# Lichtso/contrast_renderer

Hardware: AMD Instinct MI355X
Metric: paths/sec, 10k mixed-Bezier paths @ 4096^2 (tessellate + tile raster) (higher is better)
Workload: dtype f32

## Files before the change

contrast_renderer_amd/build.py:

```python
import os
import subprocess
import sys

HERE = os.path.dirname(os.path.abspath(__file__))
CSRC = os.path.join(HERE, "csrc")
SOURCES = ("tessellate.hip", "raster.hip", "bin_edges.hip", "raster_edges.hip", "image_filter.hip", "api.hip", "image.hip", "comm.hip", "text.cpp", "path.cpp")
FLAGS = ["--offload-arch=gfx950", "-O3", "-std=c++17", "-ffp-contract=off", "-fno-fast-math", "-fPIC", "-Wall", "-Wno-unused-function", "-Wno-bitwise-instead-of-logical"]
FILE_FLAGS = {"raster_edges.hip": ["-fno-slp-vectorize"], "bin_edges.hip": ["-fno-slp-vectorize", "-mllvm", "-disable-machine-licm"], "raster.hip": ["-fno-slp-vectorize", "-mllvm", "-pragma-unroll-threshold=65536"], "tessellate.hip": ["-fno-slp-vectorize"]}
OUT = os.path.join(HERE, "libcontrast_hip.so")


def _newer(target, deps):
    if not os.path.exists(target):
        return False
    t = os.path.getmtime(target)
    return all(os.path.getmtime(d) <= t for d in deps if os.path.exists(d))


def header_deps():
    own = sorted(os.path.join(CSRC, f) for f in os.listdir(CSRC) if f.endswith((".hpp", ".h", ".inc")))
    return own + [os.path.join(HERE, "..", "include", h) for h in ("contrast_hip.h", "crh_fmath.h")]


def file_flags():
# ... 18 lines not shown
        objects.append(obj)
        if not force and _newer(obj, [os.path.join(CSRC, src)] + headers):
            continue
        flags = (FLAGS + os.environ.get("CRH_EXTRA_FLAGS", "").split()) if src.endswith(".hip") else [f for f in FLAGS if not f.startswith("--offload-arch")]
        flags = flags + file_flags().get(src, [])
        cmd = [hipcc] + flags + ["-c", os.path.join(CSRC, src), "-o", obj]
        if verbose:
            print(" ".join(cmd), file=sys.stderr)
        procs.append((src, subprocess.Popen(cmd, stdout=subprocess.PIPE, stderr=subprocess.STDOUT)))
    for src, proc in procs:
        out, _ = proc.communicate()
        if proc.returncode != 0:
            raise RuntimeError(f"hipcc failed on {src}:\n{out.decode()}")
        if verbose and out:
            print(out.decode(), file=sys.stderr)
    exports = write_export_map()
    if procs or not os.path.exists(OUT) or os.path.getmtime(exports) > os.path.getmtime(OUT):
        cmd = [hipcc, "--offload-arch=gfx950", "-shared", "-fPIC"] + objects + ["-ldl", "-Wl,--version-script=" + exports, "-o", OUT]
        subprocess.check_call(cmd)
    return OUT


DEBUG_TAPS = ("crh_debug_frame_counters", "crh_debug_frame_counters16", "crh_debug_frame_words", "crh_debug_frame_bin_dump", "crh_debug_flat_batches", "crh_debug_pass_leaves_state",
              "crh_debug_frame_last_pass")


def declared_entry_points():
    import re
    with open(os.path.join(HERE, "..", "include", "contrast_hip.h")) as f:
        return sorted(set(re.findall(r"\b(crh_[a-z_0-9]+)\s*\(", f.read())) - {"crh_status"})


def write_export_map():
    path = os.path.join(HERE, "build", "exports.map")
    os.makedirs(os.path.dirname(path), exist_ok=True)
    text = "{\n  global:\n" + "".join(f"    {name};\n" for name in declared_entry_points() + list(DEBUG_TAPS)) + "  local:\n    *;\n};\n"
    if not os.path.exists(path) or open(path).read() != text:
        with open(path, "w") as f:
            f.write(text)
    return path


if __name__ == "__main__":
    print(build_library(force="--force" in sys.argv, verbose=True))
```

contrast_renderer_amd/csrc/api.hip:

```cpp
#include <hip/hip_runtime.h>

#include <algorithm>
#include <atomic>
#include <chrono>
#include <cmath>
#include <cstdio>
#include <cstdlib>
#include <cstring>
#include <memory>
#include <string>
#include <vector>

#include "api_internal.hpp"
#include "launch.hpp"
#include "raster_params.hpp"
#include "scene.hpp"

using namespace crh;

namespace {
thread_local std::string g_error;

struct DevBuf {
    void* p = nullptr;
// ... 2604 lines not shown
    return CRH_OK;
}
extern "C" crh_status crh_debug_frame_last_pass(crh_frame* f, uint32_t out[4]) {
    if (!f || !out) return CRH_ERR_INVALID_ARGUMENT;
    out[0] = f->last_formulation, out[1] = f->last_general, out[2] = f->last_raster, out[3] = f->last_bin;
    const crh_frame::BinSet& set = f->sets[f->last_set];
    if ((f->last_bin & kBinReplayed) && set.used && set.flags_host && hipEventQuery(set.flags_ready) == hipSuccess && set.flags_host[kReplayFallbackWord] != 0u) out[3] |= kBinFellBack;
    return CRH_OK;
}
extern "C" crh_status crh_debug_frame_words(crh_frame* f, uint32_t out[128]) {
    HIP_TRY(hipSetDevice(f->renderer->device));
    HIP_TRY(f->renderer->sync());
    HIP_TRY(hipMemcpy(out, f->sets[f->last_set].overflow_p, 512, hipMemcpyDeviceToHost));
    HIP_TRY(hipMemset(static_cast<uint8_t*>(f->sets[f->last_set].overflow_p) + 320, 0, 192));
    return CRH_OK;
}
extern "C" crh_status crh_debug_frame_bin_dump(crh_frame* f, uint32_t* out, uint32_t n_words) {
    HIP_TRY(hipSetDevice(f->renderer->device));
    HIP_TRY(f->renderer->sync());
    if ((size_t)n_words * 4 > f->item_cost.cap) return CRH_ERR_INVALID_ARGUMENT;
    HIP_TRY(hipMemcpy(out, f->item_cost.p, (size_t)n_words * 4, hipMemcpyDeviceToHost));
    return CRH_OK;
}
extern "C" int crh_debug_flat_batches(const uint32_t* cost, uint32_t n_items, uint32_t* runs, uint32_t cap_runs, uint32_t limits[4]) {
    std::vector<uint32_t> out;
    flat_batches(cost, n_items, out);
    flat_batch_limits(n_items, limits);
    if (out.size() / 2 > cap_runs) return -1;
    std::copy(out.begin(), out.end(), runs);
    return (int)(out.size() / 2);
}
crh_status crh_frame_device_pointer(crh_frame* f, void** out) {
    if (!f || !out) return CRH_ERR_INVALID_ARGUMENT;
    crh_status st = settle_frame(f);
    if (st != CRH_OK) return st;
    HIP_TRY(hipSetDevice(f->renderer->device));
    HIP_TRY(order_after_external(f, f->renderer->stream));
    if (f->cleared)
        HIP_TRY(hipMemsetAsync(f->rgba8.p, 0, f->image_bytes(), f->renderer->stream));
    HIP_TRY(hipStreamSynchronize(f->renderer->stream));
    *out = f->rgba8.p;
    return CRH_OK;
}
crh_status crh_internal_frame_geometry(crh_frame* f, uint32_t* width, uint32_t* height, uint32_t* format, int* device) {
    if (!f || !f->renderer || !width || !height || !format || !device) return CRH_ERR_INVALID_ARGUMENT;
    *width = f->width, *height = f->height, *format = f->format, *device = f->renderer->device;
// ... 192 lines not shown
```

contrast_renderer_amd/csrc/bin_edges.hip:

```cpp
#include <algorithm>
#include <type_traits>
#include <vector>

#include "edge_slots.hpp"
#include "launch.hpp"

namespace crh {

struct ItemCtx {
    uint32_t shape, instance, dyn0;
    uint32_t lv0, jn0, iq0, ic0, rq0, rc0, hull0, sv0;
    uint32_t cb[8];
    float m0, m4, m12, m1, m5, m13;
    float col[4];
};
CRH_D ItemCtx item_ctx(const SceneDev& s, const RasterParams& r, const DrawItem& it, const uint32_t cb[8]) {
    ItemCtx c;
    const uint32_t* b0 = s.shape_base + it.shape * kShapeRow;
    c.shape = it.shape, c.instance = it.instance, c.dyn0 = s.shape_dyn_begin[it.shape];
    c.lv0 = b0[CH_LINE_V], c.jn0 = b0[CH_JOINT], c.iq0 = b0[CH_IQ], c.ic0 = b0[CH_IC_V], c.rq0 = b0[CH_RQ], c.rc0 = b0[CH_RC_V], c.hull0 = b0[CH_HULL], c.sv0 = b0[CH_SOLID_V];
#pragma unroll
    for (int i = 0; i < 8; ++i) c.cb[i] = cb[i];
    const float* m = r.transforms + 16u * it.instance;
    c.m0 = m[0], c.m4 = m[4], c.m12 = m[12], c.m1 = m[1], c.m5 = m[5], c.m13 = m[13];
// ... 39 lines not shown
    if (s.n_shapes) hipLaunchKernelGGL(k_shape_bounds, dim3((s.n_shapes + 255u) / 256u), dim3(256), 0, stream, s, bounds);
}
__global__ __launch_bounds__(256) void k_slab_items(RasterParams r, uint8_t* elsewhere) {
    const uint32_t item = blockIdx.x * 256u + threadIdx.x;
    if (item < r.n_items) elsewhere[item] = item_misses_slab(r, item_of(r, item)) ? 1u : 0u;
}
void launch_slab_items(const RasterParams& r, uint8_t* elsewhere, hipStream_t stream) {
    if (r.n_items) hipLaunchKernelGGL(k_slab_items, dim3((r.n_items + 255u) / 256u), dim3(256), 0, stream, r, elsewhere);
}
__global__ __launch_bounds__(256) void k_item_nslots(SceneDev s, RasterParams r, uint32_t n_items, uint32_t* out) {
    const uint32_t i = blockIdx.x * 256u + threadIdx.x;
    if (i >= n_items) return;
    out[i] = item_slots(s, item_of(r, i)).total;
}

struct PlainTri {
    float2 p[3];
    float attr[3][4];
    uint32_t kind, flat_u, desc;
    float end_y;
    int n_attr;
    bool valid;
};
CRH_D void load_plain_triangle(const SceneDev& s, const ItemCtx& ctx, uint32_t c, PlainTri& out) {
    const uint32_t* cb = ctx.cb;
    const uint32_t dyn0 = ctx.dyn0;
    float2 p[3];
    float attr[3][4] = {};
    uint32_t kind, flat_u = 0, desc = 0;
    float end_y = 0.0f;
    int n_attr;
    bool valid = true;
    if (c < cb[0]) {
        const uint32_t lv0 = ctx.lv0, k = c;
        valid = s.line_pair_cut[(lv0 + k) >> 1] == 0;
        const uint32_t i0 = lv0 + k, i1 = lv0 + ((k & 1u) ? k + 2u : k + 1u), i2 = lv0 + ((k & 1u) ? k + 1u : k + 2u);
        const Vertex2f1i a = s.line_v[i0], b = s.line_v[i1], d = s.line_v[i2];
        p[0] = make_float2(a.x, a.y), p[1] = make_float2(b.x, b.y), p[2] = make_float2(d.x, d.y);
        attr[0][0] = a.u, attr[0][1] = a.v, attr[1][0] = b.u, attr[1][1] = b.v, attr[2][0] = d.u, attr[2][1] = d.v;
        flat_u = a.i;
        end_y = a.v;
        desc = dyn0 + (a.i & 65535u);
        kind = KIND_LINE;
        n_attr = 2;
    } else if (c < cb[1]) {
        const uint32_t q = c - cb[0], jn = q / 3u, k = q - 3u * jn, base = 5u * (ctx.jn0 + jn);
// ... 40 lines not shown
#pragma unroll
        for (int v = 0; v < 3; ++v) {
            const Vertex4f a = s.rc_v[at + v];
            p[v] = make_float2(a.x, a.y);
            attr[v][0] = a.k, attr[v][1] = a.l, attr[v][2] = a.m, attr[v][3] = a.n;
        }
        kind = KIND_RC;
        n_attr = 4;
    } else {
        const uint32_t k = c - cb[6], hull0 = ctx.hull0;
        const Vertex0 a = s.hull_v[hull0 + k], b = s.hull_v[hull0 + ((k & 1u) ? k + 2u : k + 1u)], d = s.hull_v[hull0 + ((k & 1u) ? k + 1u : k + 2u)];
        p[0] = make_float2(a.x, a.y), p[1] = make_float2(b.x, b.y), p[2] = make_float2(d.x, d.y);
        kind = EK_COVER_TRI;
        n_attr = 0;
    }
#pragma unroll
    for (int v = 0; v < 3; ++v) {
        out.p[v] = p[v];
#pragma unroll
        for (int a = 0; a < 4; ++a) out.attr[v][a] = attr[v][a];
    }
    out.kind = kind, out.flat_u = flat_u, out.desc = desc, out.end_y = end_y, out.n_attr = n_attr, out.valid = valid;
}
CRH_D bool place_plain_triangle(const RasterParams& r, const ItemCtx& ctx, PlainTri& t, float& det_out, ushort4& box) {
    const float W = (float)r.width, H = (float)r.height;
    float2* p = t.p;
#pragma unroll
    for (int v = 0; v < 3; ++v) p[v] = to_framebuffer(ctx, W, H, p[v].x, p[v].y);
    const float d1x = p[1].x - p[0].x, d1y = p[1].y - p[0].y;
    const float d2x = p[2].x - p[0].x, d2y = p[2].y - p[0].y;
    const float det = d1x * d2y - d2x * d1y;
    det_out = det;
    if (!(t.valid && det != 0.0f && det == det && is_finite(det))) return false;
    const float minx = fminf(p[0].x, fminf(p[1].x, p[2].x)), maxx = fmaxf(p[0].x, fmaxf(p[1].x, p[2].x));
    const float miny = fminf(p[0].y, fminf(p[1].y, p[2].y)), maxy = fmaxf(p[0].y, fmaxf(p[1].y, p[2].y));
    const bool nan_free = minx == minx && maxx == maxx && miny == miny && maxy == maxy;
    const int x0 = (int)floorf(fminf(fmaxf(minx, 0.0f), W)), x1 = (int)floorf(fmaxf(fminf(maxx, W - 1.0f), -1.0f));
    const int y0 = (int)floorf(fminf(fmaxf(miny, 0.0f), H)), y1 = (int)floorf(fmaxf(fminf(maxy, H - 1.0f), -1.0f));
    if (!(nan_free && x0 <= x1 && y0 <= y1)) return false;
    box = make_ushort4((unsigned short)x0, (unsigned short)x1, (unsigned short)y0, (unsigned short)y1);
    return true;
}
CRH_D void plain_triangle_coverage(const PlainTri& t, float det, PrimCoverage& cov) {
    const float2* p = t.p;
    const bool front = det < 0.0f;
    const float2 nv[3] = {p[0], det < 0.0f ? p[2] : p[1], det < 0.0f ? p[1] : p[2]};
// ... 121 lines not shown
    if (r.debug & 512u) return;
#endif
    if ((ballot >> lane) & 1ull) {
        const uint32_t at = st.used + lanes_below(ballot, lane);
        st.tile[at] = tile;
        st.pos[at] = pos;
        st.key[at] = key;
    }
    st.used += (uint32_t)__popcll(ballot);
    if (st.used > st.cap - 64u) {
        if (RESERVED) stage_flush_reserved(st, r, lane); else stage_flush(st, r, lane);
    }
}

CRH_D bool accepts(float e, uint32_t tl) { return e > 0.0f || (e == 0.0f && tl != 0u); }

struct BinEdge {
    float lo_x, lo_y, hi_x, hi_y, bx, nay, ymin, ymax;
    uint32_t tl, hull;
    int sigma, down;
    bool valid;
    float strip_det;
};
CRH_D BinEdge load_edge(const SceneDev& s, const RasterParams& r, const ItemCtx& ctx, uint32_t n_fe, uint32_t n_hull_chain, uint32_t i) {
    BinEdge e = {};
    e.valid = false;
    if (i >= n_fe + n_hull_chain) return e;
    float2 a, b;
    if (i < n_fe) {
        const uint32_t sv0 = ctx.sv0, g = sv0 + i, g_last = sv0 + n_fe - 1u;
        const uint32_t gm1 = i >= 1u ? g - 1u : g, gm2 = i >= 2u ? g - 2u : g, gp1 = min(g + 1u, g_last), gp2 = min(g + 2u, g_last);
        const uint32_t f = s.solid_flag[g], f_prev = s.solid_flag[gm1], f_next = s.solid_flag[gp1];
        const Vertex0 va = s.solid_v[g], vm1 = s.solid_v[gm1], vm2 = s.solid_v[gm2], vp1 = s.solid_v[gp1], vp2 = s.solid_v[gp2];
        const bool odd = (f & 1u) != 0u, last = (f & 2u) != 0u;
        const bool first = !odd && (i == 0u || (f_prev & 2u) != 0u);
        Vertex0 vb;
        if (first) {
            if (last) return e;
            vb = vp1;
        } else if (!odd) {
            vb = vm2;
        } else {
            vb = last ? vm1 : ((f_next & 2u) ? vp1 : vp2);
        }
        a = make_float2(va.x, va.y), b = make_float2(vb.x, vb.y);
    } else {
// ... 18 lines not shown
        }
    }
    const float W = (float)r.width, H = (float)r.height;
    a = to_framebuffer(ctx, W, H, a.x, a.y);
    b = to_framebuffer(ctx, W, H, b.x, b.y);
    if (!(is_finite(a.x) && is_finite(a.y) && is_finite(b.x) && is_finite(b.y))) {
        r.overflow[7] = 1u;
        return e;
    }
    if (a.x == b.x && a.y == b.y) return e;
    const bool flip = !(a.x < b.x || (a.x == b.x && a.y < b.y));
    const float2 lo = flip ? b : a, hi = flip ? a : b;
    e.lo_x = lo.x, e.lo_y = lo.y, e.hi_x = hi.x, e.hi_y = hi.y;
    e.bx = hi.x - lo.x;
    e.nay = -(hi.y - lo.y);
    const float dx = hi.x - lo.x, dy = hi.y - lo.y;
    e.tl = (dy < 0.0f || (dy == 0.0f && dx > 0.0f)) ? 1u : 0u;
    e.down = dy > 0.0f ? 1 : 0;
    e.sigma = flip ? 1 : -1;
    e.ymin = fminf(lo.y, hi.y), e.ymax = fmaxf(lo.y, hi.y);
    e.valid = true;
    return e;
}
CRH_D float wave_min(float v) {
#pragma unroll
    for (int d = 32; d > 0; d >>= 1) v = fminf(v, __shfl_xor(v, d, 64));
    return v;
}
CRH_D float wave_max(float v) {
#pragma unroll
    for (int d = 32; d > 0; d >>= 1) v = fmaxf(v, __shfl_xor(v, d, 64));
    return v;
}
CRH_D uint32_t wave_max_u32(uint32_t v) {
#pragma unroll
    for (int d = 32; d > 0; d >>= 1) v = max(v, (uint32_t)__shfl_xor((int)v, d, 64));
    return v;
}

struct TileTest {
    float bx[3], nay[3], lo_x[3], lo_y[3];
    float s_lo, s_hi;
    uint32_t tl;
    CRH_D void set(const PrimCoverage& cov, float lo, float hi) {
#pragma unroll
        for (int i = 0; i < 3; ++i) bx[i] = cov.bx[i], nay[i] = cov.nay[i], lo_x[i] = cov.lo_x[i], lo_y[i] = cov.lo_y[i];
// ... 448 lines not shown
}


#ifndef CRH_FLAT_WAVES
#define CRH_FLAT_WAVES 4
#endif
#ifndef CRH_FLAT_ROUNDS
#define CRH_FLAT_ROUNDS 3
#endif
#ifndef CRH_FLAT_STAGE
#define CRH_FLAT_STAGE 64
#endif
#ifndef CRH_FLAT_THREADS
#define CRH_FLAT_THREADS 128
#endif
constexpr uint32_t kFlatThreads = CRH_FLAT_THREADS, kFlatWaveCount = kFlatThreads / 64u;
static_assert(kFlatThreads == 64u || kFlatThreads == 128u || kFlatThreads == 256u, "CRH_FLAT_THREADS: 64, 128 or 256");
#ifndef CRH_FLAT_POOL
#define CRH_FLAT_POOL 6
#endif
#ifndef CRH_FLAT_BATCH
#define CRH_FLAT_BATCH (CRH_FLAT_THREADS / 8)
#endif
#ifndef CRH_FLAT_HITS
#define CRH_FLAT_HITS 400
#endif
constexpr uint32_t kHitIndexBits = 9, kHitCellBits = 10, kHitKeyBits = 32u - kHitIndexBits - kHitCellBits;
constexpr uint32_t kFlatItems = 32, kFlatBatch = CRH_FLAT_BATCH, kFlatTris = kFlatThreads, kFlatEdgeRounds = CRH_FLAT_ROUNDS, kFlatEdges = kFlatThreads * kFlatEdgeRounds, kFlatPool = CRH_FLAT_POOL * kFlatThreads, kFlatStage = CRH_FLAT_STAGE;
static_assert(kFlatBatch >= 1u && kFlatBatch <= kFlatItems, "CRH_FLAT_BATCH");
constexpr uint32_t kFiOpaque = 1u, kFiSkip = 2u, kFiHullTris = 4u, kFiQueue = 8u;
struct FlatItem {
    ItemCtx ctx;
    uint32_t slot0, fe_slot0, synth_a, hull_slot0, synth_b;
    uint32_t n_tri, n_fe, n_hull, n_hull_chain;
    uint32_t flags;
    int box[4];
    uint32_t faces;
    uint32_t tx_a, ty_a, tx_b, ty_b, nx, n_rect;
};
CRH_D int ordered_int(float f) {
    const int i = __float_as_int(f);
    return i ^ ((i >> 31) & 0x7FFFFFFF);
}
CRH_D float ordered_float(int i) { return __int_as_float(i ^ ((i >> 31) & 0x7FFFFFFF)); }
CRH_D uint32_t wave_inclusive_scan(uint32_t v, uint32_t lane) {
#pragma unroll
// ... 99 lines not shown
    static_assert(kFlatLds <= 160u * 1024u / kFlatGroupsPerCu / kLdsBlock * kLdsBlock, "k_bin_flat's LDS tables keep it from CRH_FLAT_WAVES wavefronts per SIMD (one workgroup per CU less where it replays)");
    const uint32_t tid0 = threadIdx.x;
    uint32_t turn = 0;
    const float ry_first = S == 1 ? 0.5f : 0.125f, r_last = (float)(kTile - 1) + (S == 1 ? 0.5f : 0.875f);
    const uint32_t first_item = r.bin_batches ? r.bin_batches[2u * blockIdx.x] : blockIdx.x * items_per_group;
    const uint32_t last_item = r.bin_batches ? r.bin_batches[2u * blockIdx.x + 1u] : min(r.n_items, first_item + items_per_group);
    const bool all_queued = (r.debug & (1u | 2u | 4194304u)) != 0u;
#ifdef CRH_ABLATE
    unsigned long long phase_t = __builtin_amdgcn_s_memtime();
    const unsigned long long born_t = phase_t;
    uint32_t dump_items = 0, dump_tris = 0, dump_edges = 0, dump_pool = 0, dump_work = 0, dump_walk = 0, dump_wave_hits = 0, dump_batch_hits = 0;
#endif
    for (uint32_t next = first_item; next < last_item;) {
        const uint32_t tid = per_turn_v(tid0), lane = tid & 63u, wave = tid >> 6;
        Stage st = {stage_tile[wave], stage_pos[wave], stage_key[wave], 0u, 0u, kFlatStage, 0xFFFFFFFFu};
        RasterParams rt = r;
        rt.width = per_turn_s(r.width), rt.height = per_turn_s(r.height);
        const float W = (float)rt.width, H = (float)rt.height;
        lds_barrier();
        const uint32_t n_cand = min(kFlatBatch, last_item - next);
        if (kReplay && tid == 0u) replay_off = 0u;
        if (tid < n_cand) {
            const uint32_t item = next + tid;
            const DrawItem it = item_of(r, item);
            const bool elsewhere = r.item_elsewhere && r.item_elsewhere[item] != 0u;
            const ItemSlots k = item_slots(s, it);
            FlatItem& fi = items[tid];
            fi.ctx = item_ctx(s, r, it, k.cb);
            const uint32_t slot0 = r.slot_begin[item];
            fi.slot0 = slot0, fi.fe_slot0 = slot0 + k.fe0, fi.synth_a = slot0 + k.synth_a, fi.hull_slot0 = slot0 + k.hull0, fi.synth_b = slot0 + k.synth_b;
            fi.n_tri = k.n_tri, fi.n_fe = k.n_fe, fi.n_hull = k.n_hull, fi.n_hull_chain = k.n_hull;
            const float* c = fi.ctx.col;
            const bool opaque = c[3] == 1.0f && is_finite(c[0]) && is_finite(c[1]) && is_finite(c[2]) && r.occlude != 0u && (r.debug & 32768u) == 0u;
            const bool oversize = k.n_tri > kFlatTris || k.n_fe + k.n_hull > kFlatEdges || all_queued || slot0 + k.total > r.slot_capacity;
            fi.flags = (opaque ? kFiOpaque : 0u) | ((oversize || elsewhere) ? kFiSkip : 0u) | ((oversize && !elsewhere && slot0 + k.total <= r.slot_capacity) ? kFiQueue : 0u);
            fi.box[0] = fi.box[1] = 0x7FFFFFFF, fi.box[2] = fi.box[3] = (int)0x80000000;
            fi.faces = 0u;
            fi.n_rect = 0u;
        }
        lds_barrier();
        if (wave == 0u) {
            const FlatItem& mine_ = items[min(lane, kFlatBatch - 1u)];
            const bool real = lane < n_cand && lane < kFlatBatch, counted = real && (mine_.flags & kFiSkip) == 0u;
            const uint32_t nt = counted ? mine_.n_tri : 0u, ne = counted ? mine_.n_fe + mine_.n_hull : 0u;
            const uint32_t pt = wave_inclusive_scan(nt, lane), pe = wave_inclusive_scan(ne, lane);
            const unsigned long long fits = __ballot(real && pt <= kFlatTris && pe <= kFlatEdges);
            const uint32_t n_batch = (uint32_t)__builtin_ctzll(~fits);
            if (lane <= kFlatItems) {
                tri_begin[lane] = lane <= n_batch ? pt - nt : 0xFFFFFFFFu;
                edge_begin[lane] = lane <= n_batch ? pe - ne : 0xFFFFFFFFu;
            }
            const uint32_t total_t = (uint32_t)__shfl((int)pt, (int)n_batch - 1, 64), total_e = (uint32_t)__shfl((int)pe, (int)n_batch - 1, 64);
            if (lane == 0u) {
                batch[0] = n_batch, batch[1] = total_t, batch[2] = total_e;
                tri_begin[n_batch] = 0xFFFFFFFFu, edge_begin[n_batch] = 0xFFFFFFFFu;
            }
        }
        lds_barrier();
        const uint32_t n_batch = batch[0], n_tris = batch[1], n_edges = batch[2];
        CRH_FLAT_PHASE(0)
#pragma unroll
        for (int k = 0; k < (int)kFlatEdgeRounds; ++k) {
            const uint32_t e = tid + kFlatThreads * (uint32_t)k;
            if (e < n_edges) {
                const uint32_t j = find_item(edge_begin, e), i = e - edge_begin[j];
                const FlatItem& fi = items[j];
                const BinEdge loaded = load_edge(s, rt, fi.ctx, fi.n_fe, fi.n_hull, i);
                edge_table[e] = pack_edge(loaded);
                edge_flags[e] = (uint16_t)pack_edge_flags(loaded, j);
            }
        }
        CRH_FLAT_PHASE(1)
        FlatTri tri;
        tri.nt = 0u, tri.item = 0u, tri.key = 0u, tri.bx0 = tri.bx1 = tri.by0 = 0u;
        tri.test = TileTest{};
        PlainTri corners;
        corners.valid = false;
        if (tid < n_tris) {
            const uint32_t j = find_item(tri_begin, tid), t = tid - tri_begin[j];
            const FlatItem& fi = items[j];
            const ItemCtx& ctx = fi.ctx;
            const uint32_t c = t < ctx.cb[1] ? t : t - ctx.cb[1] + ctx.cb[2];
            load_plain_triangle(s, ctx, c, corners);
            tri.key = fi.slot0 + 4u * t, tri.item = j;
        }
#ifdef CRH_ABLATE
        const bool store_records = (r.debug & 8388608u) == 0u;
#else
        constexpr bool store_records = true;
#endif
        if (tid < n_tris) {
            FlatItem& fi = items[tri.item];
            float det;
            ushort4 box;
            if (place_plain_triangle(rt, fi.ctx, corners, det, box)) {
                PrimRec* out = reinterpret_cast<PrimRec*>(r.slots + (size_t)tri.key * 32u);
                {
                    PrimCoverage cov;
                    cov.box = box;
                    plain_triangle_coverage(corners, det, cov);
                    tri.test.set(cov, ry_first, r_last);
                    tri.bx0 = box.x / kTile, tri.bx1 = box.y / kTile, tri.by0 = box.z / kTile;
                    tri.nt = (tri.bx1 - tri.bx0 + 1u) * (box.w / kTile - tri.by0 + 1u);
                    atomicMin(&fi.box[0], ordered_int((float)box.x)), atomicMin(&fi.box[1], ordered_int((float)box.z));
                    atomicMax(&fi.box[2], ordered_int((float)box.y)), atomicMax(&fi.box[3], ordered_int((float)box.w));
                    if (store_records) out->cov = cov;
                }
                PrimFragment frag;
// ... 237 lines not shown
            for (uint32_t w = 0; w < kFlatWaveCount; ++w) {
                const uint32_t n = hit_count[w];
                together += n;
                replay = replay && n <= replay_cap;
            }
            replay = replay && together <= hit_room;
            replay = __builtin_amdgcn_readfirstlane((int)replay) != 0;
            if (!replay && tid == 0u) atomicAdd(&r.overflow[kReplayFallbackWord], 1u);
        }
        CRH_FLAT_PHASE(5)
        constexpr uint32_t kChunks = kFlatPool / kFlatThreads;
#pragma unroll 1
        for (uint32_t ch = 0; ch * kFlatThreads < n_pool; ++ch) {
            const uint32_t p = ch * kFlatThreads + tid;
            if (p < n_pool) {
                const uint32_t j = find_item(pool_begin, p);
                const uint32_t q = p - pool_begin[j], nx = items[j].nx;
                if (q % nx == 0u)
                    for (uint32_t c = 1; c < nx; ++c) pool_back[p + c] += pool_back[p + c - 1u];
            }
        }
        lds_barrier();
        uint32_t my_synth = 0, my_opaque = 0;
        {
            uint32_t reserved[kChunks], lefts[kChunks];
#pragma unroll
            for (uint32_t ch = 0; ch < kChunks; ++ch) {
                reserved[ch] = 0u, lefts[ch] = 0u;
                const uint32_t p = ch * kFlatThreads + tid;
                if (p >= n_pool) continue;
                const uint32_t j = find_item(pool_begin, p);
                const FlatItem& fi = items[j];
                const uint32_t q = p - pool_begin[j], qy = q / fi.nx, qx = q - qy * fi.nx;
                const uint32_t tile = (fi.ty_a + qy) * r.tiles_x + fi.tx_a + qx;
                const int both = pool_back[p], bd = (int)(short)(both & 0xFFFF), hbd = (both - bd) >> 16;
                const uint32_t counted = pool_cursor[p];
                const uint32_t n_touching = counted & 0x000FFFFFu;
                const bool hull_touch = (counted >> 20) != 0u;
                const uint32_t abd = (uint32_t)(bd < 0 ? -bd : bd), ahbd = (uint32_t)(hbd < 0 ? -hbd : hbd);
                const bool cover = fi.n_hull_chain != 0u && (hbd != 0 || hull_touch);
                const int cbd = bd > 0 ? 1 : (bd < 0 ? -1 : 0), chbd = hbd > 0 ? 1 : (hbd < 0 ? -1 : 0);
                const bool hull_over_tile = cover && hbd != 0 && !hull_touch;
                const bool replaces_tile = hull_over_tile && (fi.flags & kFiOpaque) != 0u && n_touching == 0u && (bd & (int)r.winding_mask) != 0;
                const uint32_t n_bd = cover ? (abd ? abd - 1u : 0u) : abd, n_hbd = cover ? (ahbd ? ahbd - 1u : 0u) : 0u;
                const uint32_t left = (cover ? 1u : 0u) + n_bd + n_hbd;
                lefts[ch] = left;
                my_synth += left;
                my_opaque += replaces_tile ? 1u : 0u;
                if (left + n_touching) reserved[ch] = atomicAdd(&r.tile_count[tile], left + n_touching);
                pool_back[p] = (int)(left | (n_bd << 12) | (cover ? 1u << 24 : 0u) | (cbd > 0 ? 1u << 25 : 0u) | (chbd > 0 ? 1u << 26 : 0u) | (cbd < 0 ? 1u << 27 : 0u) | (chbd < 0 ? 1u << 28 : 0u) |
                                     (replaces_tile ? 1u << 29 : 0u) | (hull_over_tile ? 1u << 30 : 0u));
            }
#pragma unroll
            for (uint32_t ch = 0; ch < kChunks; ++ch)
                if (ch * kFlatThreads + tid < n_pool) pool_cursor[ch * kFlatThreads + tid] = reserved[ch] + lefts[ch];
        }
        {
            uint32_t a = my_entries, b = my_synth | (my_opaque << 22);
#pragma unroll
            for (int d = 32; d > 0; d >>= 1) a += (uint32_t)__shfl_xor((int)a, d, 64), b += (uint32_t)__shfl_xor((int)b, d, 64);
            if (lane == 0u) wave_entries[wave] = a, wave_entries[kFlatWaveCount + wave] = b & 0x003FFFFFu, wave_opaque[wave] = b >> 22;
        }
        lds_barrier();
        if (tid == 0u) {
            uint32_t total = 0;
            for (uint32_t w = 0; w < 2u * kFlatWaveCount; ++w) total += wave_entries[w];
#ifdef CRH_ABLATE
            {
                uint32_t hits = 0;
                for (uint32_t w = 0; w < kFlatWaveCount; ++w) hits += wave_entries[w], dump_wave_hits = max(dump_wave_hits, wave_entries[w]);
                dump_batch_hits = max(dump_batch_hits, hits);
            }
#endif
            uint32_t opaque = 0;
            for (uint32_t w = 0; w < kFlatWaveCount; ++w) opaque += wave_opaque[w];
            if (opaque) atomicAdd(&r.overflow[4], opaque);
            const uint32_t sub = ((blockIdx.x + 40503u * turn) * 2654435761u) >> 26, region = r.pair_capacity / kSubStreams;
            uint32_t begin = 0xFFFFFFFFu;
            if (r.direct) {
                begin = 0u;
            } else if (total) {
                const uint32_t got = atomicAdd(&r.pair_cursor[sub], total);
                if (got + total > region)
                    r.overflow[5] = 1u;
                else
                    begin = sub * region + got;
            }
            for (uint32_t w = 0; w < kFlatWaveCount; ++w) {
                const uint32_t mine = wave_entries[kFlatWaveCount + w] + wave_entries[w];
                wave_entries[w] = begin;
                if (begin != 0xFFFFFFFFu) begin += mine;
            }
        }
        lds_barrier();
        st.at = wave_entries[wave];
#pragma unroll 1
        for (uint32_t ch = 0; ch * kFlatThreads < n_pool; ++ch) {
            const uint32_t p = ch * kFlatThreads + tid;
            const bool active = p < n_pool;
            const uint32_t j = active ? find_item(pool_begin, p) : 0u;
            const FlatItem& fi = items[j];
            const uint32_t q = active ? p - pool_begin[j] : 0u, row_len = max(fi.nx, 1u), qy = q / row_len, qx = q - qy * row_len;
            const uint32_t tile = (fi.ty_a + qy) * r.tiles_x + fi.tx_a + qx;
            const uint32_t verdict = active ? (uint32_t)pool_back[p] : 0u;
            const uint32_t cbd1 = 1u + ((verdict >> 25) & 1u) - ((verdict >> 27) & 1u), chbd1 = 1u + ((verdict >> 26) & 1u) - ((verdict >> 28) & 1u);
            const uint32_t cover_key = fi.synth_b + cbd1 + 3u * chbd1 + ((verdict >> 29) & 1u ? kCoverOpaque : ((verdict >> 30) & 1u ? kCoverHull : 0u));
            const uint32_t bd_key = fi.synth_a + ((verdict >> 25) & 1u ? 0u : 1u), hbd_key = fi.synth_a + ((verdict >> 26) & 1u ? 2u : 3u);
            uint32_t left = verdict & 4095u, n_bd = (verdict >> 12) & 4095u, pos = active ? pool_cursor[p] - left : 0u;
            bool cover = (verdict >> 24) & 1u;
            if (replay && active) pool_back[p] = (int)tile;
            for (;;) {
                const unsigned long long ballot = __ballot(left != 0u);
                if (!ballot) break;
                uint32_t key = 0;
                if (left) {
                    if (cover)
                        cover = false, key = cover_key;
                    else if (n_bd)
                        --n_bd, key = bd_key;
                    else
                        key = hbd_key;
                }
                stage_append<true>(st, r, lane, ballot, tile, pos, key);
                if (left) ++pos, --left;
            }
        }
        lds_barrier();
        CRH_FLAT_PHASE(6)
        if (replay) {
            stage_flush_reserved(st, r, lane);
            for (uint32_t i = lane; i < n_hits; i += 64u) {
                const uint32_t rec = *hit_slot(i), cell = (rec >> kHitIndexBits) & ((1u << kHitCellBits) - 1u);
                const uint32_t tile = (uint32_t)pool_back[cell], pos = pool_cursor[cell] + (rec & ((1u << kHitIndexBits) - 1u)), key = key0 + (rec >> (kHitIndexBits + kHitCellBits));
#ifdef CRH_ABLATE
                if (r.debug & 512u) continue;
#endif
                if (r.direct) {
                    const uint32_t place = r.tile_base[tile];
                    if (pos < r.tile_base[tile + 1u] - place && place + pos < r.pair_capacity) r.tile_list[place + pos] = key;
                    else r.overflow[0] = 1u;
                } else if (st.at != 0xFFFFFFFFu) {
                    r.pair_tile[st.at + i] = tile, r.pair_pos[st.at + i] = pos, r.pair_key[st.at + i] = key;
                }
            }
            if (st.at != 0xFFFFFFFFu) st.at += n_hits;
        } else {
        for_edge_rows([&](bool active, const BinEdge& e, uint32_t j, const FlatItem& fi, int ty, int x0, int x1, uint32_t key) {
            const uint32_t base = pool_begin[j] + ((uint32_t)ty - fi.ty_a) * fi.nx, tx_a = fi.tx_a;
            const uint32_t cols = wave_max_u32(active && x0 <= x1 ? (uint32_t)(x1 - x0 + 1) : 0u);
            for (uint32_t c = 0; c < cols; ++c) {
                const int tx = x0 + (int)c;
                const bool hit = active && tx <= x1 && matters(e, tx, ty);
                const unsigned long long ballot = __ballot(hit);
                if (ballot) {
                    uint32_t pos = 0;
                    if (hit) pos = atomicAdd(&pool_cursor[base + ((uint32_t)tx - tx_a)], 1u);
                    stage_append<true>(st, r, lane, ballot, (uint32_t)ty * r.tiles_x + (uint32_t)tx, pos, key);
                }
            }
        });
// ... 260 lines not shown
```

Before: 40.98 million.

## Batch global loads for edges, triangles, items and write synth cells directly

```diff
diff --git a/contrast_renderer_amd/build.py b/contrast_renderer_amd/build.py
--- a/contrast_renderer_amd/build.py
+++ b/contrast_renderer_amd/build.py
@@ -64,7 +64,7 @@
 
 
 DEBUG_TAPS = ("crh_debug_frame_counters", "crh_debug_frame_counters16", "crh_debug_frame_words", "crh_debug_frame_bin_dump", "crh_debug_flat_batches", "crh_debug_pass_leaves_state",
-              "crh_debug_frame_last_pass")
+              "crh_debug_frame_last_pass", "crh_debug_frame_tile_place")
 
 
 def declared_entry_points():
diff --git a/contrast_renderer_amd/csrc/api.hip b/contrast_renderer_amd/csrc/api.hip
--- a/contrast_renderer_amd/csrc/api.hip
+++ b/contrast_renderer_amd/csrc/api.hip
@@ -2650,6 +2650,14 @@
     HIP_TRY(hipMemcpy(out, f->item_cost.p, (size_t)n_words * 4, hipMemcpyDeviceToHost));
     return CRH_OK;
 }
+extern "C" crh_status crh_debug_frame_tile_place(crh_frame* f, uint32_t tile, uint32_t out[3]) {
+    if (!f || !out || !f->direct_ready || tile >= f->n_tiles || !f->sets[f->last_set].used) return CRH_ERR_INVALID_ARGUMENT;
+    HIP_TRY(hipSetDevice(f->renderer->device));
+    HIP_TRY(f->renderer->sync());
+    HIP_TRY(hipMemcpy(out, (f->base_cur ? f->tile_base_b : f->tile_base).as<uint32_t>() + tile, 8, hipMemcpyDeviceToHost));
+    HIP_TRY(hipMemcpy(out + 2, f->sets[f->last_set].tile_count_cursor.as<uint32_t>() + f->n_tiles + tile, 4, hipMemcpyDeviceToHost));
+    return CRH_OK;
+}
 extern "C" int crh_debug_flat_batches(const uint32_t* cost, uint32_t n_items, uint32_t* runs, uint32_t cap_runs, uint32_t limits[4]) {
     std::vector<uint32_t> out;
     flat_batches(cost, n_items, out);
diff --git a/contrast_renderer_amd/csrc/bin_edges.hip b/contrast_renderer_amd/csrc/bin_edges.hip
--- a/contrast_renderer_amd/csrc/bin_edges.hip
+++ b/contrast_renderer_amd/csrc/bin_edges.hip
@@ -85,6 +85,90 @@
     int n_attr;
     bool valid;
 };
+#ifndef CRH_BIN_LOADS_TRIS
+#define CRH_BIN_LOADS_TRIS 1
+#endif
+template <class T>
+CRH_D void held(T& v) {
+#if defined(__HIP_DEVICE_COMPILE__)
+    static_assert(sizeof(T) == 4, "one vector register");
+    asm volatile("" : "+v"(v));
+#endif
+}
+#if CRH_BIN_LOADS_TRIS
+struct __attribute__((may_alias)) WordPair {
+    float a, b;
+};
+struct TriRaw {
+    WordPair xy[3], mid[3], end[3];
+    uint32_t cut, which;
+};
+CRH_D uint32_t tri_stride(uint32_t which) {
+    return which == 6u ? 2u : (which == 2u ? 4u : ((which == 1u || which == 5u) ? 6u : 5u));
+}
+CRH_D void issue_plain_triangle(const SceneDev& s, const ItemCtx& ctx, uint32_t c, TriRaw& raw) {
+    const uint32_t* cb = ctx.cb;
+    const uint32_t which = (c >= cb[0] ? 1u : 0u) + (c >= cb[1] ? 1u : 0u) + (c >= cb[3] ? 1u : 0u) + (c >= cb[4] ? 1u : 0u) + (c >= cb[5] ? 1u : 0u) + (c >= cb[6] ? 1u : 0u);
+    const uint32_t q = c - cb[0], jn = q / 3u, jk = q - 3u * jn;
+    const uint32_t first = which == 0u ? ctx.lv0 + c
+                         : which == 1u ? 5u * (ctx.jn0 + jn) + jk
+                         : which == 2u ? 3u * (ctx.iq0 + (c - cb[2]))
+                         : which == 3u ? ctx.ic0 + 3u * (c - cb[3])
+                         : which == 4u ? 3u * (ctx.rq0 + (c - cb[4]))
+                         : which == 5u ? ctx.rc0 + 3u * (c - cb[5])
+                                       : ctx.hull0 + (c - cb[6]);
+    const uint32_t odd = which == 0u ? (c & 1u) : (which == 1u ? (jk & 1u) : (which == 6u ? ((c - cb[6]) & 1u) : 0u));
+    const float* base = which == 0u ? reinterpret_cast<const float*>(s.line_v)
+                      : which == 1u ? reinterpret_cast<const float*>(s.joint_v)
+                      : which == 2u ? reinterpret_cast<const float*>(s.iq_v)
+                      : which == 3u ? reinterpret_cast<const float*>(s.ic_v)
+                      : which == 4u ? reinterpret_cast<const float*>(s.rq_v)
+                      : which == 5u ? reinterpret_cast<const float*>(s.rc_v)
+                                    : reinterpret_cast<const float*>(s.hull_v);
+    const uint32_t stride = tri_stride(which), mid = min(2u, stride - 2u), end = min(4u, stride - 2u);
+    const uint32_t at[3] = {first, first + 1u + odd, first + 2u - odd};
+#pragma unroll
+    for (int v = 0; v < 3; ++v) {
+        const float* pv = base + (size_t)at[v] * stride;
+        raw.xy[v] = *reinterpret_cast<const WordPair*>(pv);
+        raw.mid[v] = *reinterpret_cast<const WordPair*>(pv + mid);
+        raw.end[v] = *reinterpret_cast<const WordPair*>(pv + end);
+    }
+    raw.cut = 0u;
+    if (which == 0u) raw.cut = s.line_pair_cut[(ctx.lv0 + c) >> 1];
+    raw.which = which;
+}
+CRH_D void hold_plain_triangle(TriRaw& raw) {
+#pragma unroll
+    for (int v = 0; v < 3; ++v) held(raw.xy[v].a), held(raw.xy[v].b), held(raw.mid[v].a), held(raw.mid[v].b), held(raw.end[v].a), held(raw.end[v].b);
+    held(raw.cut);
+}
+CRH_D void finish_plain_triangle(const ItemCtx& ctx, const TriRaw& raw, PlainTri& out) {
+    const uint32_t which = raw.which, stride = tri_stride(which);
+    const int n_attr = which == 6u ? 0 : (which == 5u ? 4 : ((which == 0u || which == 2u) ? 2 : 3));
+    const bool stroke = which <= 1u;
+#pragma unroll
+    for (int v = 0; v < 3; ++v) {
+        out.p[v] = make_float2(raw.xy[v].a, raw.xy[v].b);
+        out.attr[v][0] = n_attr > 0 ? raw.mid[v].a : 0.0f;
+        out.attr[v][1] = n_attr > 1 ? raw.mid[v].b : 0.0f;
+        out.attr[v][2] = n_attr > 2 ? (stride == 6u ? raw.end[v].a : raw.end[v].b) : 0.0f;
+        out.attr[v][3] = n_attr > 3 ? raw.end[v].b : 0.0f;
+    }
+    out.flat_u = stroke ? __float_as_uint(raw.end[0].b) : 0u;
+    out.end_y = which == 0u ? raw.mid[0].b : 0.0f;
+    out.desc = stroke ? ctx.dyn0 + (out.flat_u & 65535u) : 0u;
+    out.kind = which == 0u ? (uint32_t)KIND_LINE : which == 1u ? (uint32_t)KIND_JOINT : which == 2u ? (uint32_t)KIND_IQ : which == 3u ? (uint32_t)KIND_IC : which == 4u ? (uint32_t)KIND_RQ : which == 5u ? (uint32_t)KIND_RC : EK_COVER_TRI;
+    out.n_attr = n_attr;
+    out.valid = raw.cut == 0u;
+}
+CRH_D void load_plain_triangle(const SceneDev& s, const ItemCtx& ctx, uint32_t c, PlainTri& out) {
+    TriRaw raw;
+    issue_plain_triangle(s, ctx, c, raw);
+    hold_plain_triangle(raw);
+    finish_plain_triangle(ctx, raw, out);
+}
+#else
 CRH_D void load_plain_triangle(const SceneDev& s, const ItemCtx& ctx, uint32_t c, PlainTri& out) {
     const uint32_t* cb = ctx.cb;
     const uint32_t dyn0 = ctx.dyn0;
@@ -171,6 +255,7 @@
     }
     out.kind = kind, out.flat_u = flat_u, out.desc = desc, out.end_y = end_y, out.n_attr = n_attr, out.valid = valid;
 }
+#endif
 CRH_D bool place_plain_triangle(const RasterParams& r, const ItemCtx& ctx, PlainTri& t, float& det_out, ushort4& box) {
     const float W = (float)r.width, H = (float)r.height;
     float2* p = t.p;
@@ -338,6 +423,103 @@
     bool valid;
     float strip_det;
 };
+#ifndef CRH_BIN_LOADS_EDGES
+#define CRH_BIN_LOADS_EDGES 1
+#endif
+#if CRH_BIN_LOADS_EDGES
+struct EdgeFlags {
+    uint32_t f, f_prev, f_next;
+};
+CRH_D EdgeFlags load_edge_flags(const SceneDev& s, const ItemCtx& ctx, uint32_t n_fe, uint32_t i, bool fill) {
+    EdgeFlags o = {0u, 0u, 0u};
+    if (fill) {
+        const uint32_t g = ctx.sv0 + i, g_last = ctx.sv0 + n_fe - 1u;
+        o.f = s.solid_flag[g], o.f_prev = s.solid_flag[i >= 1u ? g - 1u : g], o.f_next = s.solid_flag[min(g + 1u, g_last)];
+    }
+    return o;
+}
+CRH_D void hold_edge_flags(EdgeFlags& o) { held(o.f), held(o.f_prev), held(o.f_next); }
+constexpr uint32_t kEwHull = 1u, kEwStrip = 2u, kEwNone = 4u;
+struct EdgeWhere {
+    const Vertex0* v;
+    uint32_t a, b, c1, c2, bits;
+};
+CRH_D EdgeWhere edge_where(const SceneDev& s, const ItemCtx& ctx, uint32_t n_fe, uint32_t n_hull_chain, uint32_t i, const EdgeFlags& fl) {
+    const bool fill = i < n_fe;
+    const uint32_t g = ctx.sv0 + i, g_last = ctx.sv0 + n_fe - 1u;
+    const uint32_t gm1 = i >= 1u ? g - 1u : g, gm2 = i >= 2u ? g - 2u : g, gp1 = min(g + 1u, g_last), gp2 = min(g + 2u, g_last);
+    const bool odd = (fl.f & 1u) != 0u, last = (fl.f & 2u) != 0u;
+    const bool first = !odd && (i == 0u || (fl.f_prev & 2u) != 0u);
+    const uint32_t fill_b = first ? gp1 : (!odd ? gm2 : (last ? gm1 : ((fl.f_next & 2u) ? gp1 : gp2)));
+    const uint32_t pos = i - n_fe, n = n_hull_chain, hull0 = ctx.hull0;
+    const uint32_t target = pos == 0u ? 1u : ((pos & 1u) == 0u ? pos - 2u : (pos + 1u == n ? pos - 1u : (pos + 2u == n ? pos + 1u : pos + 2u)));
+    const bool strip = !fill && pos + 2u < n;
+    EdgeWhere w;
+    w.v = fill ? s.solid_v : s.hull_v;
+    w.a = fill ? g : hull0 + pos;
+    w.b = fill ? fill_b : hull0 + target;
+    w.c1 = strip ? hull0 + ((pos & 1u) ? pos + 2u : pos + 1u) : w.a;
+    w.c2 = strip ? hull0 + ((pos & 1u) ? pos + 1u : pos + 2u) : w.a;
+    w.bits = (fill ? 0u : kEwHull) | (strip ? kEwStrip : 0u) | ((fill && first && last) ? kEwNone : 0u);
+    return w;
+}
+struct EdgeVerts {
+    Vertex0 a, b, c1, c2;
+};
+CRH_D EdgeVerts load_edge_verts(const EdgeWhere& w, bool active) {
+    EdgeVerts o = {};
+    if (active) o.a = w.v[w.a], o.b = w.v[w.b], o.c1 = w.v[w.c1], o.c2 = w.v[w.c2];
+    return o;
+}
+CRH_D void hold_edge_verts(EdgeVerts& o) { held(o.a.x), held(o.a.y), held(o.b.x), held(o.b.y), held(o.c1.x), held(o.c1.y), held(o.c2.x), held(o.c2.y); }
+CRH_D BinEdge finish_edge(const RasterParams& r, const ItemCtx& ctx, uint32_t bits, const EdgeVerts& v) {
+    BinEdge e = {};
+    e.valid = false;
+    if (bits & kEwNone) return e;
+    float2 a = make_float2(v.a.x, v.a.y), b = make_float2(v.b.x, v.b.y);
+    const float W = (float)r.width, H = (float)r.height;
+    if (bits & kEwHull) {
+        e.hull = 1u;
+        if (bits & kEwStrip) {
+            const float2 p0 = to_framebuffer(ctx, W, H, v.a.x, v.a.y), p1 = to_framebuffer(ctx, W, H, v.c1.x, v.c1.y), p2 = to_framebuffer(ctx, W, H, v.c2.x, v.c2.y);
+            const float d1x = p1.x - p0.x, d1y = p1.y - p0.y, d2x = p2.x - p0.x, d2y = p2.y - p0.y;
+            const float det = d1x * d2y - d2x * d1y;
+            e.strip_det = (det == det && is_finite(det)) ? det : 0.0f;
+        }
+    }
+    a = to_framebuffer(ctx, W, H, a.x, a.y);
+    b = to_framebuffer(ctx, W, H, b.x, b.y);
+    if (!(is_finite(a.x) && is_finite(a.y) && is_finite(b.x) && is_finite(b.y))) {
+        r.overflow[7] = 1u;
+        return e;
+    }
+    if (a.x == b.x && a.y == b.y) return e;
+    const bool flip = !(a.x < b.x || (a.x == b.x && a.y < b.y));
+    const float2 lo = flip ? b : a, hi = flip ? a : b;
+    e.lo_x = lo.x, e.lo_y = lo.y, e.hi_x = hi.x, e.hi_y = hi.y;
+    e.bx = hi.x - lo.x;
+    e.nay = -(hi.y - lo.y);
+    const float dx = hi.x - lo.x, dy = hi.y - lo.y;
+    e.tl = (dy < 0.0f || (dy == 0.0f && dx > 0.0f)) ? 1u : 0u;
+    e.down = dy > 0.0f ? 1 : 0;
+    e.sigma = flip ? 1 : -1;
+    e.ymin = fminf(lo.y, hi.y), e.ymax = fmaxf(lo.y, hi.y);
+    e.valid = true;
+    return e;
+}
+CRH_D BinEdge load_edge(const SceneDev& s, const RasterParams& r, const ItemCtx& ctx, uint32_t n_fe, uint32_t n_hull_chain, uint32_t i) {
+    const bool active = i < n_fe + n_hull_chain;
+    EdgeFlags fl = load_edge_flags(s, ctx, n_fe, i, active && i < n_fe);
+    hold_edge_flags(fl);
+    const EdgeWhere w = edge_where(s, ctx, n_fe, n_hull_chain, i, fl);
+    EdgeVerts v = load_edge_verts(w, active);
+    hold_edge_verts(v);
+    BinEdge e = {};
+    e.valid = false;
+    if (active) e = finish_edge(r, ctx, w.bits, v);
+    return e;
+}
+#else
 CRH_D BinEdge load_edge(const SceneDev& s, const RasterParams& r, const ItemCtx& ctx, uint32_t n_fe, uint32_t n_hull_chain, uint32_t i) {
     BinEdge e = {};
     e.valid = false;
@@ -402,6 +584,7 @@
     e.valid = true;
     return e;
 }
+#endif
 CRH_D float wave_min(float v) {
 #pragma unroll
     for (int d = 32; d > 0; d >>= 1) v = fminf(v, __shfl_xor(v, d, 64));
@@ -896,6 +1079,12 @@
 #ifndef CRH_FLAT_BATCH
 #define CRH_FLAT_BATCH (CRH_FLAT_THREADS / 8)
 #endif
+#ifndef CRH_BIN_LOADS_ITEMS
+#define CRH_BIN_LOADS_ITEMS 1
+#endif
+#ifndef CRH_BIN_LOADS_DIRECT
+#define CRH_BIN_LOADS_DIRECT 1
+#endif
 #ifndef CRH_FLAT_HITS
 #define CRH_FLAT_HITS 400
 #endif
@@ -1041,8 +1230,14 @@
         if (kReplay && tid == 0u) replay_off = 0u;
         if (tid < n_cand) {
             const uint32_t item = next + tid;
+#if CRH_BIN_LOADS_ITEMS
+            const uint8_t* const elsewhere_at = r.item_elsewhere ? r.item_elsewhere + item : reinterpret_cast<const uint8_t*>(r.slot_begin + item);
+            const uint32_t elsewhere_byte = *elsewhere_at;
+            const DrawItem it = item_of(r, item);
+#else
             const DrawItem it = item_of(r, item);
             const bool elsewhere = r.item_elsewhere && r.item_elsewhere[item] != 0u;
+#endif
             const ItemSlots k = item_slots(s, it);
             FlatItem& fi = items[tid];
             fi.ctx = item_ctx(s, r, it, k.cb);
@@ -1051,6 +1246,9 @@
             fi.n_tri = k.n_tri, fi.n_fe = k.n_fe, fi.n_hull = k.n_hull, fi.n_hull_chain = k.n_hull;
             const float* c = fi.ctx.col;
             const bool opaque = c[3] == 1.0f && is_finite(c[0]) && is_finite(c[1]) && is_finite(c[2]) && r.occlude != 0u && (r.debug & 32768u) == 0u;
+#if CRH_BIN_LOADS_ITEMS
+            const bool elsewhere = r.item_elsewhere && elsewhere_byte != 0u;
+#endif
             const bool oversize = k.n_tri > kFlatTris || k.n_fe + k.n_hull > kFlatEdges || all_queued || slot0 + k.total > r.slot_capacity;
             fi.flags = (opaque ? kFiOpaque : 0u) | ((oversize || elsewhere) ? kFiSkip : 0u) | ((oversize && !elsewhere && slot0 + k.total <= r.slot_capacity) ? kFiQueue : 0u);
             fi.box[0] = fi.box[1] = 0x7FFFFFFF, fi.box[2] = fi.box[3] = (int)0x80000000;
@@ -1078,6 +1276,64 @@
         lds_barrier();
         const uint32_t n_batch = batch[0], n_tris = batch[1], n_edges = batch[2];
         CRH_FLAT_PHASE(0)
+        FlatTri tri;
+        tri.nt = 0u, tri.item = 0u, tri.key = 0u, tri.bx0 = tri.bx1 = tri.by0 = 0u;
+        tri.test = TileTest{};
+        PlainTri corners;
+        corners.valid = false;
+#if CRH_BIN_LOADS_TRIS
+        TriRaw tri_raw = {};
+#endif
+#if CRH_BIN_LOADS_EDGES
+        {
+            uint32_t edge_item[kFlatEdgeRounds], edge_bits[kFlatEdgeRounds];
+            EdgeFlags edge_fl[kFlatEdgeRounds];
+            EdgeVerts edge_v[kFlatEdgeRounds];
+#pragma unroll
+            for (int k = 0; k < (int)kFlatEdgeRounds; ++k) {
+                const uint32_t e = tid + kFlatThreads * (uint32_t)k;
+                const bool active = e < n_edges;
+                const uint32_t j = active ? find_item(edge_begin, e) : 0u, i = e - edge_begin[j];
+                const FlatItem& fi = items[j];
+                edge_item[k] = j;
+                edge_fl[k] = load_edge_flags(s, fi.ctx, fi.n_fe, i, active && i < fi.n_fe);
+            }
+#pragma unroll
+            for (int k = 0; k < (int)kFlatEdgeRounds; ++k) hold_edge_flags(edge_fl[k]);
+#pragma unroll
+            for (int k = 0; k < (int)kFlatEdgeRounds; ++k) {
+                const uint32_t e = tid + kFlatThreads * (uint32_t)k, j = edge_item[k];
+                const FlatItem& fi = items[j];
+                const EdgeWhere w = edge_where(s, fi.ctx, fi.n_fe, fi.n_hull, e - edge_begin[j], edge_fl[k]);
+                edge_bits[k] = w.bits;
+                edge_v[k] = load_edge_verts(w, e < n_edges);
+            }
+#if CRH_BIN_LOADS_TRIS
+            if (tid < n_tris) {
+                const uint32_t j = find_item(tri_begin, tid), t = tid - tri_begin[j];
+                const FlatItem& fi = items[j];
+                const ItemCtx& ctx = fi.ctx;
+                const uint32_t c = t < ctx.cb[1] ? t : t - ctx.cb[1] + ctx.cb[2];
+                issue_plain_triangle(s, ctx, c, tri_raw);
+                tri.key = fi.slot0 + 4u * t, tri.item = j;
+            }
+#endif
+#pragma unroll
+            for (int k = 0; k < (int)kFlatEdgeRounds; ++k) hold_edge_verts(edge_v[k]);
+#if CRH_BIN_LOADS_TRIS
+            hold_plain_triangle(tri_raw);
+#endif
+#pragma unroll
+            for (int k = 0; k < (int)kFlatEdgeRounds; ++k) {
+                const uint32_t e = tid + kFlatThreads * (uint32_t)k, j = edge_item[k];
+                if (e < n_edges) {
+                    const BinEdge loaded = finish_edge(rt, items[j].ctx, edge_bits[k], edge_v[k]);
+                    edge_table[e] = pack_edge(loaded);
+                    edge_flags[e] = (uint16_t)pack_edge_flags(loaded, j);
+                }
+            }
+        }
+#else
 #pragma unroll
         for (int k = 0; k < (int)kFlatEdgeRounds; ++k) {
             const uint32_t e = tid + kFlatThreads * (uint32_t)k;
@@ -1089,12 +1345,11 @@
                 edge_flags[e] = (uint16_t)pack_edge_flags(loaded, j);
             }
         }
+#endif
         CRH_FLAT_PHASE(1)
-        FlatTri tri;
-        tri.nt = 0u, tri.item = 0u, tri.key = 0u, tri.bx0 = tri.bx1 = tri.by0 = 0u;
-        tri.test = TileTest{};
-        PlainTri corners;
-        corners.valid = false;
+#if CRH_BIN_LOADS_TRIS && CRH_BIN_LOADS_EDGES
+        if (tid < n_tris) finish_plain_triangle(items[tri.item].ctx, tri_raw, corners);
+#else
         if (tid < n_tris) {
             const uint32_t j = find_item(tri_begin, tid), t = tid - tri_begin[j];
             const FlatItem& fi = items[j];
@@ -1103,6 +1358,7 @@
             load_plain_triangle(s, ctx, c, corners);
             tri.key = fi.slot0 + 4u * t, tri.item = j;
         }
+#endif
 #ifdef CRH_ABLATE
         const bool store_records = (r.debug & 8388608u) == 0u;
 #else
@@ -1386,11 +1642,20 @@
         }
         lds_barrier();
         uint32_t my_synth = 0, my_opaque = 0;
+        const bool direct_cells = kReplay && CRH_BIN_LOADS_DIRECT != 0 && replay && r.direct != 0u;
+        struct SynthKeys {
+            uint32_t cover, bd, hbd;
+        };
+        auto synth_keys = [&](const FlatItem& fi, uint32_t verdict) {
+            const uint32_t cbd1 = 1u + ((verdict >> 25) & 1u) - ((verdict >> 27) & 1u), chbd1 = 1u + ((verdict >> 26) & 1u) - ((verdict >> 28) & 1u);
+            return SynthKeys{fi.synth_b + cbd1 + 3u * chbd1 + ((verdict >> 29) & 1u ? kCoverOpaque : ((verdict >> 30) & 1u ? kCoverHull : 0u)),
+                             fi.synth_a + ((verdict >> 25) & 1u ? 0u : 1u), fi.synth_a + ((verdict >> 26) & 1u ? 2u : 3u)};
+        };
         {
-            uint32_t reserved[kChunks], lefts[kChunks];
+            uint32_t reserved[kChunks], lefts[kChunks], place[kChunks], place_end[kChunks];
 #pragma unroll
             for (uint32_t ch = 0; ch < kChunks; ++ch) {
-                reserved[ch] = 0u, lefts[ch] = 0u;
+                reserved[ch] = 0u, lefts[ch] = 0u, place[ch] = 0u, place_end[ch] = 0u;
                 const uint32_t p = ch * kFlatThreads + tid;
                 if (p >= n_pool) continue;
                 const uint32_t j = find_item(pool_begin, p);
@@ -1412,12 +1677,39 @@
                 my_synth += left;
                 my_opaque += replaces_tile ? 1u : 0u;
                 if (left + n_touching) reserved[ch] = atomicAdd(&r.tile_count[tile], left + n_touching);
+                if (direct_cells) place[ch] = r.tile_base[tile], place_end[ch] = r.tile_base[tile + 1u];
                 pool_back[p] = (int)(left | (n_bd << 12) | (cover ? 1u << 24 : 0u) | (cbd > 0 ? 1u << 25 : 0u) | (chbd > 0 ? 1u << 26 : 0u) | (cbd < 0 ? 1u << 27 : 0u) | (chbd < 0 ? 1u << 28 : 0u) |
                                      (replaces_tile ? 1u << 29 : 0u) | (hull_over_tile ? 1u << 30 : 0u));
             }
 #pragma unroll
+            for (uint32_t ch = 0; ch < kChunks; ++ch) held(reserved[ch]), held(place[ch]), held(place_end[ch]);
+            if (direct_cells) {
+#pragma unroll
+                for (uint32_t ch = 0; ch < kChunks; ++ch) {
+                    const uint32_t p = ch * kFlatThreads + tid;
+                    if (p >= n_pool) continue;
+                    const uint32_t base = place[ch], room = min(place_end[ch] - base, r.pair_capacity > base ? r.pair_capacity - base : 0u), limit = base + room;
+                    const uint32_t verdict = (uint32_t)pool_back[p];
+                    const SynthKeys keys = synth_keys(items[find_item(pool_begin, p)], verdict);
+                    uint32_t at = base + reserved[ch], n_bd = (verdict >> 12) & 4095u;
+                    bool cover = (verdict >> 24) & 1u, outgrown = false;
+                    for (uint32_t left = lefts[ch]; left != 0u; --left, ++at) {
+                        uint32_t key = keys.hbd;
+                        if (cover)
+                            cover = false, key = keys.cover;
+                        else if (n_bd)
+                            --n_bd, key = keys.bd;
+                        if (at < limit) r.tile_list[at] = key;
+                        else outgrown = true;
+                    }
+                    if (outgrown) r.overflow[0] = 1u;
+                    pool_cursor[p] = at, pool_back[p] = (int)limit;
+                }
+            } else {
+#pragma unroll
             for (uint32_t ch = 0; ch < kChunks; ++ch)
                 if (ch * kFlatThreads + tid < n_pool) pool_cursor[ch * kFlatThreads + tid] = reserved[ch] + lefts[ch];
+            }
         }
         {
             uint32_t a = my_entries, b = my_synth | (my_opaque << 22);
@@ -1459,7 +1751,7 @@
         lds_barrier();
         st.at = wave_entries[wave];
 #pragma unroll 1
-        for (uint32_t ch = 0; ch * kFlatThreads < n_pool; ++ch) {
+        for (uint32_t ch = 0; !direct_cells && ch * kFlatThreads < n_pool; ++ch) {
             const uint32_t p = ch * kFlatThreads + tid;
             const bool active = p < n_pool;
             const uint32_t j = active ? find_item(pool_begin, p) : 0u;
@@ -1467,9 +1759,8 @@
             const uint32_t q = active ? p - pool_begin[j] : 0u, row_len = max(fi.nx, 1u), qy = q / row_len, qx = q - qy * row_len;
             const uint32_t tile = (fi.ty_a + qy) * r.tiles_x + fi.tx_a + qx;
             const uint32_t verdict = active ? (uint32_t)pool_back[p] : 0u;
-            const uint32_t cbd1 = 1u + ((verdict >> 25) & 1u) - ((verdict >> 27) & 1u), chbd1 = 1u + ((verdict >> 26) & 1u) - ((verdict >> 28) & 1u);
-            const uint32_t cover_key = fi.synth_b + cbd1 + 3u * chbd1 + ((verdict >> 29) & 1u ? kCoverOpaque : ((verdict >> 30) & 1u ? kCoverHull : 0u));
-            const uint32_t bd_key = fi.synth_a + ((verdict >> 25) & 1u ? 0u : 1u), hbd_key = fi.synth_a + ((verdict >> 26) & 1u ? 2u : 3u);
+            const SynthKeys keys = synth_keys(fi, verdict);
+            const uint32_t cover_key = keys.cover, bd_key = keys.bd, hbd_key = keys.hbd;
             uint32_t left = verdict & 4095u, n_bd = (verdict >> 12) & 4095u, pos = active ? pool_cursor[p] - left : 0u;
             bool cover = (verdict >> 24) & 1u;
             if (replay && active) pool_back[p] = (int)tile;
@@ -1499,7 +1790,10 @@
 #ifdef CRH_ABLATE
                 if (r.debug & 512u) continue;
 #endif
-                if (r.direct) {
+                if (direct_cells) {
+                    if (pos < tile) r.tile_list[pos] = key;
+                    else r.overflow[0] = 1u;
+                } else if (r.direct) {
                     const uint32_t place = r.tile_base[tile];
                     if (pos < r.tile_base[tile + 1u] - place && place + pos < r.pair_capacity) r.tile_list[place + pos] = key;
                     else r.overflow[0] = 1u;
```

After: 42.72 million, median of 6. +4.2%, better.
